# JacekNaruniec/LiveScan3D

Hardware: AMD Instinct MI355X
Metric: fused frames/s (N x 512x424 depth -> merged cloud) (higher is better)
Workload: dtype f32

## Files before the change

### livescan3d_amd/csrc/fusion.hip

```cpp


#include "fusion_shared.hpp"

namespace {

struct Iv { float lo, hi; };
__device__ __forceinline__ Iv iv_scale(Iv a, float c) { const float x = a.lo * c, y = a.hi * c; return c >= 0.0f ? Iv{x, y} : Iv{y, x}; }
__device__ __forceinline__ Iv iv_shift(Iv a, float c) { return Iv{a.lo + c, a.hi + c}; }
__device__ __forceinline__ Iv iv_sum(Iv a, Iv b) { return Iv{a.lo + b.lo, a.hi + b.hi}; }
__device__ __forceinline__ bool iv_finite(Iv a) { return isfinite(a.lo) && isfinite(a.hi); }

__device__ __forceinline__ float depth_to_metres1(float d)
{
    const f2 z = depth_to_metres2(f2{d, d});
    return z.x;
}

__device__ __forceinline__ int classify_range(int a, int b, float xfac, float yfac, const SensorParams &P, const float (&bx)[6])
{
    if (a == b) {
        f2 ox, oy, oz;
        unproject2(f2{(float)a, (float)a}, f2{xfac, xfac}, f2{yfac, yfac}, P, ox, oy, oz);
        const bool rejected = (ox.x < bx[0]) | (ox.x > bx[3]) | (oy.x < bx[1]) | (oy.x > bx[4]) | (oz.x < bx[2]) | (oz.x > bx[5]);
        return rejected ? 0 : 1;
// ... 51 lines not shown
    }
}

template <bool VEC>
__device__ __forceinline__ void load_thresholds(const FuseArgs &a, const Tile &t, unsigned int (&lo)[kPxPerLane], unsigned int (&cnt)[kPxPerLane],
                                                bool &any_flagged)
{
    const int p0 = t.px0 + threadIdx.x * kPxPerLane;
    unsigned int c[kPxPerLane];
#pragma unroll
    for (int k = 0; k < kPxPerLane; k++) c[k] = 1u;
    const unsigned int *tp = a.thr + t.pix_base + p0;
    if (VEC) {
        if (p0 < t.npix) {
            const uint4 u = reinterpret_cast<const uint4 *>(tp)[0], v = reinterpret_cast<const uint4 *>(tp)[1];
            c[0] = u.x; c[1] = u.y; c[2] = u.z; c[3] = u.w; c[4] = v.x; c[5] = v.y; c[6] = v.z; c[7] = v.w;
        }
    } else {
#pragma unroll
        for (int k = 0; k < kPxPerLane; k++)
            if (p0 + k < t.npix) c[k] = tp[k];
    }
    bool fl = false;
#pragma unroll
    for (int k = 0; k < kPxPerLane; k++) {
        lo[k] = c[k] & 0xFFFFu;
        cnt[k] = c[k] >> 16;
        fl |= lo[k] == 0;
    }
    any_flagged = __any(fl);
}

__device__ __forceinline__ int wave_count_thr(const Inputs &in, const unsigned int (&lo)[kPxPerLane], const unsigned int (&cnt)[kPxPerLane])
{
    int wt = 0;
#pragma unroll
    for (int k = 0; k < kPxPerLane; k++) {
        const unsigned int d = (k & 1) ? in.dw[k >> 1] >> 16 : in.dw[k >> 1] & 0xFFFFu;
        wt += __popcll(__ballot(d - lo[k] < cnt[k]));
    }
    return wt;
}

template <bool VEC, int kTickGroup>
__global__ __launch_bounds__(kThreads) void count_thr_kernel(const FuseArgs a)
{
    __shared__ int s_cnt[4][kTickGroup];
    const int lane = threadIdx.x & 63;
    const int wave = threadIdx.x >> 6;
    const int tg = blockIdx.x / a.tiles_per_tick;
    const int tile = blockIdx.x - tg * a.tiles_per_tick;
    const int tick0 = tg * kTickGroup;
    const int nt = min(kTickGroup, a.n_ticks - tick0);
    const Tile t = locate(a, tick0, tile);
    unsigned int lo[kPxPerLane], cnt[kPxPerLane];
    bool any_flagged;
    load_thresholds<VEC>(a, t, lo, cnt, any_flagged);
    Inputs in[kTickGroup];
#pragma unroll
    for (int i = 0; i < kTickGroup; i++) {
        Tile ti = t;
        ti.dptr = t.dptr + (long long)(i < nt ? i : 0) * a.tick_depth_stride;
        load_inputs<VEC, false>(ti, in[i]);
    }
    if (!any_flagged) {
#pragma unroll
        for (int i = 0; i < kTickGroup; i++) {
            const int wt = wave_count_thr(in[i], lo, cnt);
            if (lane == 0) s_cnt[wave][i] = wt;
        }
    } else {
        const SensorParams P = a.params[t.f];
        float xf[kPxPerLane], yf[kPxPerLane];
        tile_factors<VEC>(t, xf, yf);
#pragma unroll 1
        for (int i = 0; i < nt; i++) {
            Tile ti = t;
            ti.dptr = t.dptr + (long long)i * a.tick_depth_stride;
            Inputs ix;
            load_inputs<VEC, false>(ti, ix);
            bool keep[kPxPerLane];
            uint4 unused[kPxPerLane];
            compute_pixels<false>(a, P, ix, xf, yf, keep, unused);
            int wt = 0;
#pragma unroll
            for (int k = 0; k < kPxPerLane; k++) wt += __popcll(__ballot(keep[k]));
            if (lane == 0) s_cnt[wave][i] = wt;
        }
    }
    __syncthreads();
    if ((int)threadIdx.x < nt)
        a.tile_counts[(long long)(tick0 + threadIdx.x) * a.tiles_per_tick + tile] =
            s_cnt[0][threadIdx.x] + s_cnt[1][threadIdx.x] + s_cnt[2][threadIdx.x] + s_cnt[3][threadIdx.x];
}

constexpr unsigned long long kFlagAggregate = 1ull << 62;
constexpr unsigned long long kFlagPrefix = 2ull << 62;
constexpr int kSpinLimit = 1 << 20;

constexpr int kEpochShift = 34;
constexpr unsigned long long kTileAggregate = 1ull << 32, kTilePrefix = 2ull << 32;

__device__ __forceinline__ int tile_lookback(const FuseArgs &a, int tick, int tile, int tile_tot, int lane)
{
    unsigned long long *st = a.run_state + (long long)tick * a.tiles_per_tick;
    const unsigned long long tag = (unsigned long long)a.epoch << kEpochShift;
    if (lane == 0)
        __hip_atomic_store(&st[tile], tag | (tile == 0 ? kTilePrefix : kTileAggregate) | (unsigned int)tile_tot, __ATOMIC_RELAXED,
                           __HIP_MEMORY_SCOPE_AGENT);
    int acc = 0;
    int pos = tile - 1 - lane;
    bool done = tile == 0;
    int spins = 0;
    const bool near_polls = a.n_ticks > 1;
    while (!done) {
        unsigned long long w = tag | kTilePrefix;
        if (pos >= 0) {
            if (near_polls && (spins & 3) != 3) w = __hip_atomic_load(&st[pos], __ATOMIC_RELAXED, __HIP_MEMORY_SCOPE_WORKGROUP);
            else w = __hip_atomic_load(&st[pos], __ATOMIC_RELAXED, __HIP_MEMORY_SCOPE_AGENT);
        }
        bool again = false;
        const unsigned int flag = (w >> kEpochShift) == a.epoch ? (unsigned int)(w >> 32) & 3u : 0u;
        const unsigned long long pref = __ballot(flag == 2);
        const int first = pref ? __ffsll((long long)pref) - 1 : 63;
        const unsigned long long relevant = first >= 63 ? ~0ull : ((2ull << first) - 1ull);
        const bool poisoned = (__ballot(flag == 3) & relevant) != 0;
        if (poisoned || (__ballot(flag == 0) & relevant) != 0) {
            if (poisoned || ++spins > kSpinLimit) {
                if (lane == 0) {
                    atomicExch(a.error_flag, 1);
                    if (a.offsets_mirror) a.offsets_mirror[a.n_frames + 1] = 1;
                    __hip_atomic_store(&st[tile], tag | (3ull << 32), __ATOMIC_RELAXED, __HIP_MEMORY_SCOPE_AGENT);
                }
                return -1;
            }
            __builtin_amdgcn_s_sleep(1);
            again = true;
        } else {
            acc += wave_sum(lane <= first ? (int)(unsigned int)w : 0);
            if (pref) done = true;
        }
        if (!done && !again) pos -= 64;
    }
    if (lane == 0 && tile != 0)
        __hip_atomic_store(&st[tile], tag | kTilePrefix | (unsigned int)(acc + tile_tot), __ATOMIC_RELAXED, __HIP_MEMORY_SCOPE_AGENT);
    return acc;
}


template <int MODE, bool VEC, bool LAZY = false, bool HOST = false>
__global__ __launch_bounds__(kThreads) void fuse_kernel(const FuseArgs a)
{
    constexpr bool kWrite = MODE != 0;
    __shared__ uint4 stage[kWrite ? kStageSlots : 1];
    __shared__ int s_wave_tot[4];
    __shared__ int s_wave_next[4];
    __shared__ int s_base;
    const int lane = threadIdx.x & 63;
    const int wave = threadIdx.x >> 6;
    int tick = blockIdx.x / a.tiles_per_tick;
    int tile = blockIdx.x - tick * a.tiles_per_tick;
    if (kWrite && a.chunk > 0) {
        const int per_chunk = a.chunk * a.n_ticks;
        const int chunk = blockIdx.x / per_chunk;
        const int r = blockIdx.x - chunk * per_chunk;
        const int width = min(a.chunk, a.tiles_per_tick - chunk * a.chunk);
        tick = r / width;
        tile = chunk * a.chunk + (r - tick * width);
    }
    tile += a.tile0;
    if (MODE == 1 && a.reverse_ticks) tick = a.n_ticks - 1 - tick;
    const int lin = tick * a.tiles_per_tick + tile;

    const Tile t = locate(a, tick, tile);
    Inputs in;
    load_inputs<VEC, kWrite && !LAZY>(t, in);
    Inputs nx;
    if (MODE == 3) {
        Tile tn = t;
        tn.dptr = a.depth_next + tick * a.tick_depth_stride + t.pix_base;
        load_inputs<VEC, false>(tn, nx);
    }
    const SensorParams P = a.params[t.f];
    float xf[kPxPerLane], yf[kPxPerLane];
    tile_factors<VEC>(t, xf, yf);
    bool keep[kPxPerLane];
    uint4 vert[kPxPerLane];
    compute_pixels<kWrite>(a, P, in, xf, yf, keep, vert);
    if (kWrite && LAZY) {
        bool any = false;
#pragma unroll
        for (int k = 0; k < kPxPerLane; k++) any |= keep[k];
        if (any) {
            load_rgb<VEC>(t, in);
#pragma unroll
            for (int k = 0; k < kPxPerLane; k++) vert[k].x = rgba_of(in, k);
        }
    }
    if (MODE == 3) {
        int wt = 0;
        bool arithmetic = true;
        if (a.thr) {
            unsigned int lo[kPxPerLane], cnt[kPxPerLane];
            bool any_flagged;
            load_thresholds<VEC>(a, t, lo, cnt, any_flagged);
            arithmetic = any_flagged;
            if (!any_flagged) wt = wave_count_thr(nx, lo, cnt);
        }
        if (arithmetic) {
            bool keep_n[kPxPerLane];
            uint4 unused[kPxPerLane];
            compute_pixels<false>(a, P, nx, xf, yf, keep_n, unused);
#pragma unroll
            for (int k = 0; k < kPxPerLane; k++) wt += __popcll(__ballot(keep_n[k]));
        }
        if (lane == 0) s_wave_next[wave] = wt;
    }

    int below, wave_total;
    rank_from_masks(keep, below, wave_total);
    if (lane == 0) s_wave_tot[wave] = wave_total;
    int base = 0, counted = 0;
    if (MODE == 1 || MODE == 3) {
        base = a.tile_counts[lin];
        counted = (tile + 1 < a.tiles_per_tick ? a.tile_counts[lin + 1] : a.offsets[tick * (a.n_frames + 1) + a.n_frames]) - base;
    }
    __syncthreads();
    int wave_off = 0, tile_tot = 0;
#pragma unroll
    for (int i = 0; i < 4; i++) {
        const int v = s_wave_tot[i];
        if (i < wave) wave_off += v;
        tile_tot += v;
    }
    if (MODE == 0) {
        if (threadIdx.x == 0) a.tile_counts[lin] = tile_tot;
        return;
    }
    if (MODE == 3 && threadIdx.x == 0) a.tile_counts_next[lin] = s_wave_next[0] + s_wave_next[1] + s_wave_next[2] + s_wave_next[3];
    if (MODE == 4) {
        if (wave == 0) {
            const int b = tile_lookback(a, tick, tile, tile_tot, lane);
            if (lane == 0) s_base = b;
        }
        __syncthreads();
        base = s_base;
        if (base < 0) {
            if (threadIdx.x == 0 && tile == a.tiles_per_tick - 1) {
                a.offsets[tick * (a.n_frames + 1) + a.n_frames] = -1;
                if (a.offsets_mirror) a.offsets_mirror[a.n_frames] = -1;
            }
            return;
        }
        if (threadIdx.x == 0) {
            int *off = a.offsets + tick * (a.n_frames + 1);
            if (t.frame_start) off[t.f] = base;
            if (tile == a.tiles_per_tick - 1) off[a.n_frames] = base + tile_tot;
            if (a.offsets_mirror) {
                if (t.frame_start) a.offsets_mirror[t.f] = base;
                if (tile == a.tiles_per_tick - 1) a.offsets_mirror[a.n_frames] = base + tile_tot;
            }
            if (a.group_end_mirror && blockIdx.x == gridDim.x - 1) *a.group_end_mirror = base + tile_tot;
        }
    }
    if (MODE != 4 && tile_tot != counted) {
        if (threadIdx.x == 0) atomicExch(a.error_flag, 2);
        return;
    }
    if (VEC ? a.pm_first != nullptr : a.pixmap != nullptr) {
        const int p0 = t.px0 + threadIdx.x * kPxPerLane;
        if (p0 < t.npix) {
            int r = base + wave_off + below;
            if (VEC) {
                unsigned int m = 0;
#pragma unroll
                for (int k = 0; k < kPxPerLane; k++) m |= keep[k] ? (1u << k) : 0u;
                const long long g = (tick * a.tick_depth_stride + t.pix_base + p0) >> 3;
                a.pm_first[g] = r;
                a.pm_mask[g] = (unsigned char)m;
            } else {
                int *pm = a.pixmap + tick * a.tick_depth_stride + t.pix_base + p0;
#pragma unroll
                for (int k = 0; k < kPxPerLane; k++) {
                    if (p0 + k < t.npix) pm[k] = keep[k] ? r : -1;
                    r += keep[k] ? 1 : 0;
                }
            }
        }
    }
    stage_and_store(stage, keep, vert, wave_off + below, tile_tot, a.out + tick * a.tick_vert_stride + base, HOST || (MODE == 4 && a.host_out != 0));
}



template <bool VEC>
__global__ __launch_bounds__(kThreads) void run_kernel(const FuseArgs a)
{
    __shared__ uint4 stage[kStageSlots];
    __shared__ int s_wave_tot[4];
    __shared__ int s_run;
    __shared__ int s_base;
    const int lane = threadIdx.x & 63;
    const int wave = threadIdx.x >> 6;

    const int tick = blockIdx.x % a.n_ticks;
    if (threadIdx.x == 0) s_run = (int)atomicAdd(a.ticket + 32 * tick, 1u);
    __syncthreads();
    const int run = s_run;
    if (run >= a.runs_per_tick) return;
    const int t0 = run * a.tiles_per_run;
    const int t1 = min(t0 + a.tiles_per_run, a.tiles_per_tick);

    int wave_total = 0;
    {
        Tile t = locate(a, tick, t0);
        Inputs in;
        load_inputs<VEC, false>(t, in);
        for (int tile = t0; tile < t1; tile++) {
            Tile tn = t;
            Inputs nx = in;
            if (tile + 1 < t1) {
                tn = locate(a, tick, tile + 1);
                load_inputs<VEC, false>(tn, nx);
            }
            bool counted = false;
            if (a.thr) {
                unsigned int lo[kPxPerLane], cnt[kPxPerLane];
                bool any_flagged;
                load_thresholds<VEC>(a, t, lo, cnt, any_flagged);
                if (!any_flagged) {
                    wave_total += wave_count_thr(in, lo, cnt);
                    counted = true;
                }
            }
            if (!counted) {
                bool keep[kPxPerLane];
                uint4 unused[kPxPerLane];
                compute_tile<VEC, false>(a, t, in, keep, unused);
#pragma unroll
                for (int k = 0; k < kPxPerLane; k++) wave_total += __popcll(__ballot(keep[k]));
            }
            t = tn;
            in = nx;
        }
    }
    if (lane == 0) s_wave_tot[wave] = wave_total;
    __syncthreads();
    const int run_tot = s_wave_tot[0] + s_wave_tot[1] + s_wave_tot[2] + s_wave_tot[3];

    Tile t = locate(a, tick, t0);
    Inputs in;
    load_inputs<VEC, true>(t, in);

    if (wave == 0) {
        unsigned long long *st = a.run_state + (long long)tick * a.tiles_per_tick;
        if (lane == 0) {
            const unsigned long long w = (run == 0 ? kFlagPrefix : kFlagAggregate) | (unsigned int)run_tot;
            __hip_atomic_store(&st[run], w, __ATOMIC_RELAXED, __HIP_MEMORY_SCOPE_AGENT);
        }
        int acc = 0;
        int pos = run - 1 - lane;
        bool done = run == 0;
        int spins = 0;
        while (!done) {
            unsigned long long w = kFlagPrefix;
            if (pos >= 0) w = __hip_atomic_load(&st[pos], __ATOMIC_RELAXED, __HIP_MEMORY_SCOPE_AGENT);
            const unsigned int flag = (unsigned int)(w >> 62);
            const unsigned long long pref = __ballot(flag == 2);
            const int first = pref ? __ffsll((long long)pref) - 1 : 63;
            const unsigned long long relevant = first >= 63 ? ~0ull : ((2ull << first) - 1ull);
            const unsigned long long empty = __ballot(flag == 0) & relevant;
            if (empty != 0) {
                if (++spins > kSpinLimit) {
                    if (lane == 0) atomicExch(a.error_flag, 1);
                    break;
                }
                __builtin_amdgcn_s_sleep(2);
                continue;
            }
            const int v = (lane <= first) ? (int)(unsigned int)w : 0;
            acc += wave_sum(v);
            if (pref) done = true;
            else pos -= 64;
        }
        if (lane == 0) {
            if (run != 0) {
                const unsigned long long w = kFlagPrefix | (unsigned int)(acc + run_tot);
                __hip_atomic_store(&st[run], w, __ATOMIC_RELAXED, __HIP_MEMORY_SCOPE_AGENT);
            }
            s_base = acc;
        }
    }
    __syncthreads();
    int running = s_base;

    int *off = a.offsets + (long long)tick * (a.n_frames + 1);
    for (int tile = t0; tile < t1; tile++) {
        Tile tn = t;
        Inputs nx = in;
        if (tile + 1 < t1) {
            tn = locate(a, tick, tile + 1);
            load_inputs<VEC, true>(tn, nx);
        }
        bool keep[kPxPerLane];
        uint4 vert[kPxPerLane];
        compute_tile<VEC, true>(a, t, in, keep, vert);
        int below, wave_tot2;
        rank_from_masks(keep, below, wave_tot2);
        if (lane == 0) s_wave_tot[wave] = wave_tot2;
        __syncthreads();
        int wave_off = 0, tile_tot = 0;
#pragma unroll
        for (int i = 0; i < 4; i++) {
            const int v = s_wave_tot[i];
            if (i < wave) wave_off += v;
            tile_tot += v;
        }
        if (threadIdx.x == 0 && t.frame_start) off[t.f] = running;
        if (tile_tot > 0) {
            stage_and_store(stage, keep, vert, wave_off + below, tile_tot, a.out + tick * a.tick_vert_stride + running);
        } else {
            __syncthreads();
        }
        running += tile_tot;
        t = tn;
        in = nx;
    }
    if (threadIdx.x == 0 && t1 == a.tiles_per_tick) off[a.n_frames] = running;
}


__global__ __launch_bounds__(kThreads) void table_kernel(const FrameDesc *frames, const SensorParams *params, int n_frames, float *xtab,
                                                         float *ytab)
{
    const int f = blockIdx.y;
    if (f >= n_frames) return;
    const FrameDesc fd = frames[f];
    const SensorParams P = params[f];
    for (int i = blockIdx.x * kThreads + threadIdx.x; i < fd.w + fd.h; i += gridDim.x * kThreads) {
        if (i < fd.w) xtab[fd.xtab_off + i] = ((float)i - P.cx) / P.fx;
        else ytab[fd.ytab_off + (i - fd.w)] = (P.cy - (float)(i - fd.w)) / P.fy;
    }
}
// ... 109 lines not shown
        for (auto &e : p->events) {
            (void)hipEventDestroy(e.first);
            (void)hipEventDestroy(e.second);
        }
        p->rd.destroy_event();
        if (p->side) {
            (void)hipStreamSynchronize(p->side);
            (void)hipStreamDestroy(p->side);
            (void)hipEventDestroy(p->ev_counted);
            (void)hipEventDestroy(p->ev_written[0]);
            (void)hipEventDestroy(p->ev_written[1]);
        }
        delete p;
    });
}

extern "C" long long lsnFusionTickCapacity(const LsnFusion *p) { return p ? p->cap : 0; }

extern "C" int lsnPackSensorParams(const float *intr7, const float *wt12, float *out16)
{
    return lsn::guarded("lsnPackSensorParams", -1, [&]() {
        lsn::clear_error();
        if (!intr7 || !wt12 || !out16) {
            lsn::set_error("lsnPackSensorParams: null argument");
            return -1;
        }
        SensorParams s;
        pack_sensor_params(intr7, wt12, s);
        static_assert(sizeof(SensorParams) == 16 * sizeof(float), "SensorParams is 16 floats");
        memcpy(out16, &s, sizeof(s));
        return 0;
    });
}

extern "C" int lsnFusionSetParams(LsnFusion *p, const float *intr, const float *wt, const float *bounds6, void *stream)
{
    return lsn::guarded("lsnFusionSetParams", -1, [&]() {
        lsn::clear_error();
        if (!p || !intr || !wt || !bounds6) {
            lsn::set_error("lsnFusionSetParams: null argument");
            return -1;
        }
        LSN_HIP(hipSetDevice(p->device));
        {
            std::lock_guard<std::mutex> g(p->mu);
            if (p->params_set && p->last_intr.size() == 7 * (size_t)p->n_maps &&
                memcmp(p->last_intr.data(), intr, sizeof(float) * 7 * p->n_maps) == 0 &&
                memcmp(p->last_wt.data(), wt, sizeof(float) * 12 * p->n_maps) == 0 && memcmp(p->bounds, bounds6, sizeof(p->bounds)) == 0)
                return 0;
        }
        std::vector<SensorParams> sp(p->n_maps);
        for (int i = 0; i < p->n_maps; i++) pack_sensor_params(intr + 7 * i, wt + 12 * i, sp[i]);
        LSN_HIP(hipMemcpyAsync(p->params.p, sp.data(), sizeof(SensorParams) * p->n_maps, hipMemcpyHostToDevice,
                               lsn::as_stream(stream)));
        hipLaunchKernelGGL(table_kernel, dim3(8, (unsigned)p->n_maps), dim3(kThreads), 0, lsn::as_stream(stream), p->frames.as<FrameDesc>(),
                           p->params.as<SensorParams>(), p->n_maps, p->xtab.as<float>(), p->ytab.as<float>());
        LSN_HIP(hipGetLastError());
        LSN_HIP(hipStreamSynchronize(lsn::as_stream(stream)));
        std::lock_guard<std::mutex> g(p->mu);
        memcpy(p->bounds, bounds6, sizeof(p->bounds));
        p->last_intr.assign(intr, intr + 7 * (size_t)p->n_maps);
        p->last_wt.assign(wt, wt + 12 * (size_t)p->n_maps);
        p->params_set = true;
        p->params_gen++;
        p->thr_valid = false;
        p->runs_with_params = 0;
        return 0;
    });
}

extern "C" int lsnFusionSetMode(LsnFusion *p, int mode)
{
    return lsn::guarded("lsnFusionSetMode", -1, [&]() {
        if (!p || mode < lsn::kPlanThreeLaunches || mode > lsn::kPlanSinglePass) {
            lsn::set_error("lsnFusionSetMode: mode must be 0 (count/scan/write launches), 1 (single launch, runs + look-back) or 2 (single pass, look-back per tile)");
            return -1;
        }
        p->mode = mode;
        return 0;
    });
}

extern "C" int lsnFusionSetPipelined(LsnFusion *p, int enable)
{
    return lsn::guarded("lsnFusionSetPipelined", -1, [&]() {
        lsn::clear_error();
        if (!p) return -1;
        std::lock_guard<std::mutex> g(p->mu);
        LSN_HIP(hipSetDevice(p->device));
        if (enable && !p->side) {
            if (p->tile_counts_b.reserve(sizeof(int) * (size_t)p->tiles_per_tick * p->n_ticks) ||
                p->offs_int.reserve(sizeof(int) * 2 * (size_t)p->n_ticks * (p->n_maps + 1)))
                return -1;
            LSN_HIP(hipStreamCreateWithFlags(&p->side, hipStreamNonBlocking));
            LSN_HIP(hipEventCreateWithFlags(&p->ev_counted, hipEventDisableTiming));
            LSN_HIP(hipEventCreateWithFlags(&p->ev_written[0], hipEventDisableTiming));
            LSN_HIP(hipEventCreateWithFlags(&p->ev_written[1], hipEventDisableTiming));
        }
        if (!enable && p->side) LSN_HIP(hipStreamSynchronize(p->side));
        p->pipelined = enable != 0;
        p->calls = 0;
        return 0;
    });
}

extern "C" int lsnFusionProfile(LsnFusion *p, int enable)
{
    return lsn::guarded("lsnFusionProfile", -1, [&]() {
        if (!p) return -1;
        p->profile = enable != 0;
        p->profile_every = enable > 1 ? enable : 1;
        p->profile_seq = 0;
        return 0;
    });
}

static int drain_events(LsnFusion *p)
{
    for (size_t i = 0; i < p->ev_used; i++) {
        float ms = 0;
        LSN_HIP(hipEventSynchronize(p->events[i].second));
        LSN_HIP(hipEventElapsedTime(&ms, p->events[i].first, p->events[i].second));
        p->acc_ms += ms;
        p->launches++;
    }
    p->ev_used = 0;
    return 0;
}

extern "C" int lsnFusionKernelStats(LsnFusion *p, double *avg_ms, long long *launches, char *name, int name_len, int reset)
{
    return lsn::guarded("lsnFusionKernelStats", -1, [&]() {
        lsn::clear_error();
        if (!p) return -1;
        std::lock_guard<std::mutex> g(p->mu);
        LSN_HIP(hipSetDevice(p->device));
        if (drain_events(p)) return -1;
        if (avg_ms) *avg_ms = p->launches ? p->acc_ms / (double)p->launches : 0.0;
        if (launches) *launches = p->launches;
        if (name && name_len > 0)
            snprintf(name, (size_t)name_len, "%s", p->timed_kernel ? p->timed_kernel : (p->mode == lsn::kPlanThreeLaunches ? "fuse_kernel<1>" : p->mode == lsn::kPlanSinglePass ? "fuse_kernel<4>" : "run_kernel"));
        if (reset) {
            p->acc_ms = 0;
            p->launches = 0;
        }
        return 0;
    });
}

void lsn::fill_args(LsnFusion *p, FuseArgs &a, const void *d_depth, const void *d_colors, void *d_vertices, int *d_offsets, bool with_pixmap)
{
    a.epoch = 0;
    a.chunk = 0;
    a.frames = p->frames.as<FrameDesc>();
    a.tiles = p->tile_frame.as<TileDesc>();
    a.params = p->params.as<SensorParams>();
    a.xtab = p->xtab.as<float>();
    a.ytab = p->ytab.as<float>();
    a.depth = static_cast<const unsigned short *>(d_depth);
    a.rgb = static_cast<const unsigned char *>(d_colors);
    a.out = static_cast<uint4 *>(d_vertices);
    a.tile_counts = p->tile_counts.as<int>();
    a.run_state = p->tile_state.as<unsigned long long>();
    a.error_flag = p->misc.as<int>();
    a.ticket = p->misc.as<unsigned int>() + 32;
    a.offsets = d_offsets;
    a.pixmap = with_pixmap ? p->pixmap.as<int>() : nullptr;
    a.pm_first = with_pixmap ? p->pm_first.as<int>() : nullptr;
    a.pm_mask = with_pixmap ? p->pm_mask.as<unsigned char>() : nullptr;
    a.n_frames = p->n_maps;
    a.tiles_per_tick = p->tiles_per_tick;
    a.n_ticks = p->n_ticks;
    {
        const long long total = (long long)p->tiles_per_tick * p->n_ticks;
        long long tpr = total / (6ll * 7 * 256);
        if (tpr < 1) tpr = 1;
        if (tpr > 8) tpr = 8;
        if (tpr > p->tiles_per_tick) tpr = p->tiles_per_tick;
        a.tiles_per_run = (int)tpr;
        a.runs_per_tick = (p->tiles_per_tick + a.tiles_per_run - 1) / a.tiles_per_run;
    }
    a.tick_depth_stride = p->tick_depth_elems;
    a.tick_rgb_stride = p->tick_rgb_bytes;
    a.tick_vert_stride = p->cap;
    a.minX = p->bounds[0]; a.minY = p->bounds[1]; a.minZ = p->bounds[2];
    a.maxX = p->bounds[3]; a.maxY = p->bounds[4]; a.maxZ = p->bounds[5];

    a.depth_next = nullptr;
    a.tile_counts_next = nullptr;
    a.thr = p->thr_valid ? p->thr.as<unsigned int>() : nullptr;
    a.tile0 = 0;
    a.reverse_ticks = 1;
    a.host_out = 0;
    a.offsets_mirror = nullptr;
    a.group_end_mirror = nullptr;
}

int lsn::ensure_thresholds(LsnFusion *p, hipStream_t s)
{
    if (!p->thr_enabled || p->thr_valid) return 0;
    if (++p->runs_with_params < 2) return 0;
    if (p->thr.reserve(sizeof(unsigned int) * (size_t)p->cap)) return -1;
    hipEvent_t e0, e1;
    LSN_HIP(hipEventCreate(&e0));
    LSN_HIP(hipEventCreate(&e1));
    LSN_HIP(hipEventRecord(e0, s));
    hipLaunchKernelGGL(thresh_kernel, dim3(256, (unsigned)p->n_maps), dim3(kThreads), 0, s, p->frames.as<FrameDesc>(), p->params.as<SensorParams>(),
                       p->n_maps, p->xtab.as<float>(), p->ytab.as<float>(), p->thr.as<unsigned int>(), p->bounds[0], p->bounds[1], p->bounds[2],
                       p->bounds[3], p->bounds[4], p->bounds[5]);
    LSN_HIP(hipGetLastError());
    LSN_HIP(hipEventRecord(e1, s));
    LSN_HIP(hipEventSynchronize(e1));
    (void)hipEventElapsedTime(&p->thr_build_ms, e0, e1);
    (void)hipEventDestroy(e0);
    (void)hipEventDestroy(e1);
    p->thr_valid = true;
    return 0;
}

template <int MODE, bool LAZY, bool HOST>
static void launch_fuse_as(bool vec, int grid, hipStream_t s, const FuseArgs &a)
{
    if (vec) hipLaunchKernelGGL((fuse_kernel<MODE, true, LAZY, HOST>), dim3(grid), dim3(kThreads), 0, s, a);
    else     hipLaunchKernelGGL((fuse_kernel<MODE, false, LAZY, HOST>), dim3(grid), dim3(kThreads), 0, s, a);
}

template <int MODE>
static void launch_fuse(bool vec, int grid, hipStream_t s, const FuseArgs &a, bool lazy_rgb = false, bool host_out = false)
{
    if constexpr (MODE == lsn::kPassWrite) {
        if (host_out) return launch_fuse_as<MODE, true, true>(vec, grid, s, a);
    }
    if constexpr (MODE == lsn::kPassWrite || MODE == lsn::kPassSingle) {
        if (lazy_rgb) return launch_fuse_as<MODE, true, false>(vec, grid, s, a);
    }
    launch_fuse_as<MODE, false, false>(vec, grid, s, a);
}

template <int kTickGroup>
static void launch_count_thr(bool vec, int grid, hipStream_t s, const FuseArgs &a)
{
    if (vec) hipLaunchKernelGGL((count_thr_kernel<true, kTickGroup>), dim3(grid), dim3(kThreads), 0, s, a);
    else     hipLaunchKernelGGL((count_thr_kernel<false, kTickGroup>), dim3(grid), dim3(kThreads), 0, s, a);
}

void lsn::count_and_scan(LsnFusion *p, bool vec, hipStream_t s, const FuseArgs &a, int *mirror)
{
    if (a.thr) {
        const int G = a.n_ticks >= 8 ? 8 : (a.n_ticks >= 4 ? 4 : 1);
        const int grid = p->tiles_per_tick * ((a.n_ticks + G - 1) / G);
        if (G == 8) launch_count_thr<8>(vec, grid, s, a);
        else if (G == 4) launch_count_thr<4>(vec, grid, s, a);
        else launch_count_thr<1>(vec, grid, s, a);
    } else {
        launch_fuse<lsn::kPassCount>(vec, p->tiles_per_tick * a.n_ticks, s, a);
    }
    hipLaunchKernelGGL(scan_kernel, dim3((unsigned)a.n_ticks), dim3(kScanThreads), 0, s, a.tile_counts, a.tiles_per_tick, a.frames, a.n_frames, a.offsets, mirror);
}

int lsn::next_event_pair(LsnFusion *p, hipEvent_t &e0, hipEvent_t &e1)
{
    if (p->ev_used == p->events.size()) {
        if (p->events.size() >= 4096) {
            if (drain_events(p)) return -1;
        } else {
            hipEvent_t x, y;
            LSN_HIP(hipEventCreate(&x));
            LSN_HIP(hipEventCreate(&y));
            p->events.emplace_back(x, y);
        }
    }
    e0 = p->events[p->ev_used].first;
    e1 = p->events[p->ev_used].second;
    p->ev_used++;
    return 0;
}

extern "C" int lsnFusionRun(LsnFusion *p, const void *d_depth, const void *d_colors, void *d_vertices, int *d_offsets,
                            void *stream)
{
    return lsn::guarded("lsnFusionRun", -1, [&]() {
        lsn::clear_error();
        return lsn::run_vertices(p, d_depth, d_colors, d_vertices, d_offsets, lsn::as_stream(stream));
    });
}

int lsn::run_vertices(LsnFusion *p, const void *d_depth, const void *d_colors, void *d_vertices, int *d_offsets, hipStream_t s)
{
    if (!p || !d_depth || !d_colors || !d_vertices || !d_offsets) {
        lsn::set_error("lsnFusionRun: null argument");
        return -1;
    }
    std::lock_guard<std::mutex> g(p->mu);
    return lsn::run_locked(p, d_depth, d_colors, d_vertices, d_offsets, s, false);
}

static int next_epoch(LsnFusion *p, hipStream_t s)
{
    if (p->epoch == 0 || p->epoch >= (1u << 30) - 1) {
        LSN_HIP(hipMemsetAsync(p->tile_state.p, 0, sizeof(unsigned long long) * (size_t)p->tiles_per_tick * p->n_ticks, s));
        p->epoch = 0;
    }
    ++p->epoch;
    return 0;
}


static int run_three_launches(LsnFusion *p, FuseArgs &a, bool vec, hipStream_t s, hipEvent_t e0, hipEvent_t e1)
{
    count_and_scan(p, vec, s, a);
    if (e0) LSN_HIP(hipEventRecord(e0, s));
    a.chunk = 0;
    launch_fuse<lsn::kPassWrite>(vec, p->tiles_per_tick * p->n_ticks, s, a, p->lazy_rgb);
    if (e1) LSN_HIP(hipEventRecord(e1, s));
    return 0;
}

static int run_pipelined(LsnFusion *p, FuseArgs &a, bool vec, hipStream_t s, hipEvent_t e0, hipEvent_t e1)
{
    const int b = (int)(p->calls & 1);
    const size_t off_elems = (size_t)p->n_ticks * (p->n_maps + 1);
    int *d_offsets = a.offsets, *off_int = p->offs_int.as<int>() + b * off_elems;
    a.tile_counts = b ? p->tile_counts_b.as<int>() : p->tile_counts.as<int>();
    if (p->calls >= 2) LSN_HIP(hipStreamWaitEvent(p->side, p->ev_written[b], 0));
    a.offsets = off_int;
    count_and_scan(p, vec, p->side, a);
    a.offsets = d_offsets;
    LSN_HIP(hipEventRecord(p->ev_counted, p->side));
    LSN_HIP(hipStreamWaitEvent(s, p->ev_counted, 0));
    LSN_HIP(hipMemcpyAsync(d_offsets, off_int, sizeof(int) * off_elems, hipMemcpyDeviceToDevice, s));
    if (e0) LSN_HIP(hipEventRecord(e0, s));
    launch_fuse<lsn::kPassWrite>(vec, p->tiles_per_tick * p->n_ticks, s, a);
    if (e1) LSN_HIP(hipEventRecord(e1, s));
    LSN_HIP(hipEventRecord(p->ev_written[b], s));
    p->calls++;
    return 0;
}

static int run_single_pass(LsnFusion *p, FuseArgs &a, bool vec, hipStream_t s, hipEvent_t e0, hipEvent_t e1)
{
    if (next_epoch(p, s)) return -1;
    a.epoch = p->epoch;
    constexpr int kFuseChunk = 16;
    a.chunk = kFuseChunk;
    if (e0) LSN_HIP(hipEventRecord(e0, s));
    launch_fuse<lsn::kPassSingle>(vec, p->tiles_per_tick * p->n_ticks, s, a, p->lazy_rgb);
    if (e1) LSN_HIP(hipEventRecord(e1, s));
    return 0;
}

static int run_lookback_runs(LsnFusion *p, FuseArgs &a, bool vec, hipStream_t s, hipEvent_t e0, hipEvent_t e1)
{
    LSN_HIP(hipMemsetAsync(p->tile_state.p, 0, sizeof(unsigned long long) * (size_t)p->tiles_per_tick * p->n_ticks, s));
    LSN_HIP(hipMemsetAsync(p->misc.as<char>() + 128, 0, 128 * (size_t)p->n_ticks, s));
    if (e0) LSN_HIP(hipEventRecord(e0, s));
    const int rgrid = a.runs_per_tick * p->n_ticks;
    if (vec) hipLaunchKernelGGL((run_kernel<true>), dim3(rgrid), dim3(kThreads), 0, s, a);
    else     hipLaunchKernelGGL((run_kernel<false>), dim3(rgrid), dim3(kThreads), 0, s, a);
    if (e1) LSN_HIP(hipEventRecord(e1, s));
    return 0;
}

enum class RunForm { ThreeLaunches, Pipelined, SinglePass, LookbackRuns };
static RunForm run_form(const LsnFusion *p, bool with_pixmap)
{
    switch (p->mode) {
    case lsn::kPlanThreeLaunches:
        if (p->pipelined) return with_pixmap ? RunForm::ThreeLaunches : RunForm::Pipelined;
        return p->n_ticks == 1 && p->one_tick_single_pass ? RunForm::SinglePass : RunForm::ThreeLaunches;
    case lsn::kPlanLookbackRuns:
        return with_pixmap ? RunForm::ThreeLaunches : RunForm::LookbackRuns;
    default:
        return with_pixmap ? RunForm::ThreeLaunches : RunForm::SinglePass;
    }
}

int lsn::run_locked(LsnFusion *p, const void *d_depth, const void *d_colors, void *d_vertices, int *d_offsets, hipStream_t s, bool with_pixmap)
{
    if (!p->params_set) {
        lsn::set_error("lsnFusionRun: lsnFusionSetParams has not been called");
        return -1;
    }
    if (((uintptr_t)d_vertices & 15) != 0) {
        lsn::set_error("lsnFusionRun: d_vertices must be 16-byte aligned");
        return -1;
    }
    LSN_HIP(hipSetDevice(p->device));
    if (ensure_thresholds(p, s)) return -1;
    FuseArgs a;
    fill_args(p, a, d_depth, d_colors, d_vertices, d_offsets, with_pixmap);
    const bool vec = wide_loads(p, d_depth, d_colors);

    hipEvent_t e0 = nullptr, e1 = nullptr;
    if (timed_launch(p) && next_event_pair(p, e0, e1)) return -1;

    const RunForm form = run_form(p, with_pixmap);
    if (p->mode == lsn::kPlanThreeLaunches) p->timed_kernel = form == RunForm::SinglePass ? "fuse_kernel<4>" : nullptr;
    int rc = -1;
    switch (form) {
    case RunForm::ThreeLaunches: rc = run_three_launches(p, a, vec, s, e0, e1); break;
    case RunForm::Pipelined:     rc = run_pipelined(p, a, vec, s, e0, e1); break;
    case RunForm::SinglePass:    rc = run_single_pass(p, a, vec, s, e0, e1); break;
    case RunForm::LookbackRuns:  rc = run_lookback_runs(p, a, vec, s, e0, e1); break;
    }
    if (rc) return -1;
    LSN_HIP(hipGetLastError());
    return 0;
}

int lsn::run_frames(LsnFusion *p, const void *d_depth, const void *d_colors, void *d_vertices, int *d_offsets, int f0, int f1, bool first_of_tick,
                    bool with_pixmap, int *offsets_mirror, int *group_end_mirror, bool host_out, hipStream_t s)
{
    if (!p || !d_depth || !d_colors || !d_vertices || !d_offsets || f0 < 0 || f1 > p->n_maps || f0 >= f1 || p->n_ticks != 1) {
        lsn::set_error("run_frames: bad arguments");
        return -1;
    }
    if (!p->params_set) {
        lsn::set_error("run_frames: lsnFusionSetParams has not been called");
        return -1;
    }
    std::lock_guard<std::mutex> g(p->mu);
    LSN_HIP(hipSetDevice(p->device));
    const bool vec = wide_loads(p, d_depth, d_colors);
    if (with_pixmap && reserve_pixmap(p, vec)) return -1;
    FuseArgs a;
    fill_args(p, a, d_depth, d_colors, d_vertices, d_offsets, with_pixmap);
    if (first_of_tick && next_epoch(p, s)) return -1;
    a.epoch = p->epoch;
    a.chunk = 0;
    a.tile0 = p->tile_start[f0];
    a.offsets_mirror = offsets_mirror;
    a.group_end_mirror = group_end_mirror;
    a.host_out = host_out ? 1 : 0;
    launch_fuse<lsn::kPassSingle>(vec, p->tile_start[f1] - p->tile_start[f0], s, a, p->lazy_rgb);
    LSN_HIP(hipGetLastError());
    return 0;
}

int lsn::run_count(LsnFusion *p, const void *d_depth, const void *d_colors, int *d_offsets, int *offsets_mirror, hipEvent_t counted, hipStream_t s)
{
    if (!p || !d_depth || !d_colors || !d_offsets || p->n_ticks != 1) {
        lsn::set_error("run_count: bad arguments");
        return -1;
    }
    if (!p->params_set) {
        lsn::set_error("run_count: lsnFusionSetParams has not been called");
        return -1;
    }
    std::lock_guard<std::mutex> g(p->mu);
    LSN_HIP(hipSetDevice(p->device));
    if (ensure_thresholds(p, s)) return -1;
    FuseArgs a;
    fill_args(p, a, d_depth, d_colors, nullptr, d_offsets, false);
    count_and_scan(p, wide_loads(p, d_depth, d_colors), s, a, offsets_mirror);
    LSN_HIP(hipGetLastError());
    if (counted) LSN_HIP(hipEventRecord(counted, s));
    return 0;
}

int lsn::run_write(LsnFusion *p, const void *d_depth, const void *d_colors, void *vertices, int *d_offsets, bool with_pixmap, bool host_out, hipStream_t s)
{
    if (!p || !d_depth || !d_colors || !vertices || !d_offsets || p->n_ticks != 1 || ((uintptr_t)vertices & 15) != 0) {
        lsn::set_error("run_write: bad arguments");
        return -1;
    }
    std::lock_guard<std::mutex> g(p->mu);
    LSN_HIP(hipSetDevice(p->device));
    const bool vec = wide_loads(p, d_depth, d_colors);
    if (with_pixmap && reserve_pixmap(p, vec)) return -1;
    FuseArgs a;
    fill_args(p, a, d_depth, d_colors, vertices, d_offsets, with_pixmap);
    launch_fuse<lsn::kPassWrite>(vec, p->tiles_per_tick, s, a, p->lazy_rgb, host_out);
    LSN_HIP(hipGetLastError());
    return 0;
}

extern "C" int lsnFusionRunStreamed(LsnFusion *p, const void *d_depth, const void *d_colors, void *d_vertices, int *d_offsets,
                                    const void *d_next_depth, void *stream)
{
    return lsn::guarded("lsnFusionRunStreamed", -1, [&]() {
        lsn::clear_error();
        if (!p || !d_depth || !d_colors || !d_vertices || !d_offsets) {
            lsn::set_error("lsnFusionRunStreamed: null argument");
            return -1;
        }
        if (!p->params_set) {
            lsn::set_error("lsnFusionRunStreamed: lsnFusionSetParams has not been called");
            return -1;
        }
        std::lock_guard<std::mutex> g(p->mu);
        LSN_HIP(hipSetDevice(p->device));
        hipStream_t s = lsn::as_stream(stream);
        const size_t n_tiles = (size_t)p->tiles_per_tick * p->n_ticks;
        const size_t off_elems = (size_t)p->n_ticks * (p->n_maps + 1);
        if (p->tile_counts_b.reserve(sizeof(int) * n_tiles) || p->offs_int.reserve(sizeof(int) * 2 * off_elems)) return -1;

        if (ensure_thresholds(p, s)) return -1;
// ... 80 lines not shown
```

### livescan3d_amd/csrc/fusion_shared.hpp

```cpp
#pragma once

#include "lsn_common.hpp"
#include "wave_ops.hpp"

#include <cstdint>
#include <mutex>
#include <vector>

namespace lsn {

constexpr int kPlanThreeLaunches = 0;
constexpr int kPlanLookbackRuns = 1;
constexpr int kPlanSinglePass = 2;
constexpr int kPassCount = 0;
constexpr int kPassWrite = 1;
constexpr int kPassWriteCountNext = 3;
constexpr int kPassSingle = 4;

struct FrameDesc {
    int w, h, npix, tile_start;
    long long depth_off;
    long long rgb_off;
    int xtab_off, ytab_off;
    float inv_w;
    int pad1;
};

struct TileDesc {
    int frame;
    int x0, y0;
    int pad;
};

struct SensorParams {
    float cx, cy, fx, fy;
    float t0, t1, t2;
    float r00, r01, r02, r10, r11, r12, r20, r21, r22;
};

inline void pack_sensor_params(const float *ip, const float *tp, SensorParams &s)
{
    s.cx = ip[0]; s.cy = ip[1]; s.fx = ip[2]; s.fy = ip[3];
    s.t0 = tp[0]; s.t1 = tp[1]; s.t2 = tp[2];
    s.r00 = tp[3]; s.r01 = tp[4]; s.r02 = tp[5];
    s.r10 = tp[6]; s.r11 = tp[7]; s.r12 = tp[8];
    s.r20 = tp[9]; s.r21 = tp[10]; s.r22 = tp[11];
}

struct FuseArgs {
    const FrameDesc *frames;
    const TileDesc *tiles;
    const SensorParams *params;
    const float *xtab;
    const float *ytab;
    const unsigned short *depth;
    const unsigned char *rgb;
    uint4 *out;
    int *tile_counts;
    unsigned long long *run_state;
    unsigned int *ticket;
    int *offsets;
    int *pixmap;
    int *pm_first;
    unsigned char *pm_mask;
    const unsigned short *depth_next;
    int *tile_counts_next;
    int *error_flag;
    const unsigned int *thr;
    int n_frames;
    int tiles_per_tick;
    int n_ticks;
    int tiles_per_run;
    unsigned int epoch;
    int chunk;
    int reverse_ticks;
    int tile0;
    int host_out;
    int *group_end_mirror;
    int *offsets_mirror;
    int runs_per_tick;
    long long tick_depth_stride;
    long long tick_rgb_stride;
    long long tick_vert_stride;
    float minX, minY, minZ, maxX, maxY, maxZ;
};

struct TriArgs {
    const FrameDesc *frames;
    const TileDesc *tiles;
    const unsigned short *depth;
    const int *pixmap;
    const int *pm_first;
    const unsigned char *pm_mask;
    int *tri;
    int *tile_counts;
    unsigned int *codes;
    int tiles_per_tick;
    int win;
    int host_out;
    int index_base;
    long long tick_pix_stride;
    long long tick_tri_stride;
};

}
using lsn::FrameDesc;
using lsn::FuseArgs;
using lsn::TriArgs;
using lsn::SensorParams;
using lsn::pack_sensor_params;
using lsn::TileDesc;

namespace {

constexpr int kThreads = 256;
constexpr int kPxPerLane = 8;
constexpr int kTile = kThreads * kPxPerLane;
constexpr int kWin = 1152;
constexpr bool kNontemporalStores = true;



typedef float f2 __attribute__((ext_vector_type(2)));

__device__ __forceinline__ f2 depth_to_metres2(f2 d)
{
    const f2 r = {0x1.0624dep-10f, 0x1.0624dep-10f};
    const f2 k = {1000.0f, 1000.0f};
    const f2 q0 = d * r;
    const f2 e = __builtin_elementwise_fma(-q0, k, d);
    return __builtin_elementwise_fma(e, r, q0);
}

__device__ __forceinline__ void unproject2(f2 d, f2 xfac, f2 yfac, const SensorParams &P, f2 &ox, f2 &oy, f2 &oz)
{
    f2 Z = depth_to_metres2(d);
    f2 X = xfac * Z;
    f2 Y = yfac * Z;
    X = X + P.t0;
    Y = Y + P.t1;
    Z = Z + P.t2;
    ox = X * P.r00 + Y * P.r01 + Z * P.r02;
    oy = X * P.r10 + Y * P.r11 + Z * P.r12;
    oz = X * P.r20 + Y * P.r21 + Z * P.r22;
}

__device__ __forceinline__ bool inside_box(float ox, float oy, float oz, const FuseArgs &a)
{
    const bool rejected = (ox < a.minX) | (ox > a.maxX) | (oy < a.minY) | (oy > a.maxY) | (oz < a.minZ) | (oz > a.maxZ);
    return !rejected;
}

__device__ __forceinline__ void rank_from_masks(const bool (&keep)[kPxPerLane], int &below, int &wave_total)
{
    below = 0;
    wave_total = 0;
#pragma unroll
    for (int k = 0; k < kPxPerLane; k++) {
        const unsigned long long m = __ballot(keep[k]);
        below = __builtin_amdgcn_mbcnt_hi((unsigned int)(m >> 32), __builtin_amdgcn_mbcnt_lo((unsigned int)m, below));
        wave_total += __popcll(m);
    }
}


struct Tile {
    long long pix_base;
    int f, w, h, npix, px0;
    int x0, y0;
    float inv_w;
    bool frame_start;
    const unsigned short *dptr;
    const unsigned char *cptr;
    const float *xt, *yt;
};

__device__ __forceinline__ Tile locate(const FuseArgs &a, int tick, int tile)
{
    Tile t;
    const TileDesc td = a.tiles[tile];
    t.f = td.frame;
    t.x0 = td.x0;
    t.y0 = td.y0;
    const FrameDesc fd = a.frames[t.f];
    t.inv_w = fd.inv_w;
    t.pix_base = fd.depth_off;
    t.w = fd.w;
    t.h = fd.h;
    t.npix = fd.npix;
    t.px0 = (tile - fd.tile_start) * kTile;
    t.frame_start = tile == fd.tile_start;
    t.dptr = a.depth + tick * a.tick_depth_stride + fd.depth_off;
    t.cptr = a.rgb + tick * a.tick_rgb_stride + fd.rgb_off;
    t.xt = a.xtab + fd.xtab_off;
    t.yt = a.ytab + fd.ytab_off;
    return t;
}

struct Inputs {
    unsigned int dw[4];
    unsigned int cw[6];
};

template <bool VEC, bool RGB>
__device__ __forceinline__ void load_inputs(const Tile &t, Inputs &in)
{
    const int p0 = t.px0 + threadIdx.x * kPxPerLane;
#pragma unroll
    for (int i = 0; i < 4; i++) in.dw[i] = 0;
#pragma unroll
    for (int i = 0; i < 6; i++) in.cw[i] = 0;
    if (VEC) {
        if (p0 < t.npix) {
            const uint4 dv = *reinterpret_cast<const uint4 *>(t.dptr + p0);
            in.dw[0] = dv.x; in.dw[1] = dv.y; in.dw[2] = dv.z; in.dw[3] = dv.w;
            if (RGB) {
                const uint2 *cp = reinterpret_cast<const uint2 *>(t.cptr + 3ll * p0);
                const uint2 c0 = cp[0], c1 = cp[1], c2 = cp[2];
                in.cw[0] = c0.x; in.cw[1] = c0.y; in.cw[2] = c1.x; in.cw[3] = c1.y; in.cw[4] = c2.x; in.cw[5] = c2.y;
            }
        }
    } else {
#pragma unroll
        for (int k = 0; k < kPxPerLane; k++) {
            if (p0 + k < t.npix) {
                const unsigned int d = t.dptr[p0 + k];
                in.dw[k >> 1] |= d << ((k & 1) * 16);
                if (RGB) {
                    const unsigned char *c = t.cptr + 3ll * (p0 + k);
                    const unsigned int rgb = c[0] | (c[1] << 8) | (c[2] << 16);
                    const int b = 3 * k;
                    in.cw[b >> 2] |= rgb << ((b & 3) * 8);
                    if ((b & 3) > 1) in.cw[(b >> 2) + 1] |= rgb >> ((4 - (b & 3)) * 8);
                }
            }
        }
    }
}

template <bool VEC>
__device__ __forceinline__ void load_rgb(const Tile &t, Inputs &in)
{
    const int p0 = t.px0 + threadIdx.x * kPxPerLane;
    if (VEC) {
        if (p0 < t.npix) {
            const uint2 *cp = reinterpret_cast<const uint2 *>(t.cptr + 3ll * p0);
            const uint2 c0 = cp[0], c1 = cp[1], c2 = cp[2];
            in.cw[0] = c0.x; in.cw[1] = c0.y; in.cw[2] = c1.x; in.cw[3] = c1.y; in.cw[4] = c2.x; in.cw[5] = c2.y;
        }
    } else {
#pragma unroll
        for (int k = 0; k < kPxPerLane; k++) {
            if (p0 + k < t.npix) {
                const unsigned char *c = t.cptr + 3ll * (p0 + k);
                const unsigned int rgb = c[0] | (c[1] << 8) | (c[2] << 16);
                const int b = 3 * k;
                in.cw[b >> 2] |= rgb << ((b & 3) * 8);
                if ((b & 3) > 1) in.cw[(b >> 2) + 1] |= rgb >> ((4 - (b & 3)) * 8);
            }
        }
    }
}

__device__ __forceinline__ unsigned int rgba_of(const Inputs &in, int k)
{
    const int b = 3 * k;
    const unsigned int lo = in.cw[b >> 2];
    const unsigned int hi = in.cw[(b >> 2) + 1 < 6 ? (b >> 2) + 1 : 5];
    return (__funnelshift_r(lo, hi, (b & 3) * 8) & 0x00FFFFFFu) | 0xFF000000u;
}

__device__ __forceinline__ void lane_origin(const Tile &t, int &x, int &y)
{
    const int p0 = t.px0 + threadIdx.x * kPxPerLane;
    const int v = t.x0 + (int)threadIdx.x * kPxPerLane;
    int q = (int)((float)v * t.inv_w);
    x = v - q * t.w;
    if (x < 0) { q--; x += t.w; }
    if (x >= t.w) { q++; x -= t.w; }
    y = t.y0 + q;
    if (p0 >= t.npix) { x = 0; y = 0; }
}

__device__ __forceinline__ void store_vertex(uint4 *dst, const uint4 v)
{
    if (kNontemporalStores) {
        __builtin_nontemporal_store(v.x, &dst->x);
        __builtin_nontemporal_store(v.y, &dst->y);
        __builtin_nontemporal_store(v.z, &dst->z);
        __builtin_nontemporal_store(v.w, &dst->w);
    } else {
        *dst = v;
    }
}

template <bool VEC>
__device__ __forceinline__ void tile_factors(const Tile &t, float (&xf)[kPxPerLane], float (&yf)[kPxPerLane])
{
    int x, y;
    lane_origin(t, x, y);
    float yfac = t.yt[y];
    if (VEC) {
        const float4 x0 = *reinterpret_cast<const float4 *>(t.xt + x);
        const float4 x1 = *reinterpret_cast<const float4 *>(t.xt + x + 4);
        xf[0] = x0.x; xf[1] = x0.y; xf[2] = x0.z; xf[3] = x0.w;
        xf[4] = x1.x; xf[5] = x1.y; xf[6] = x1.z; xf[7] = x1.w;
#pragma unroll
        for (int k = 0; k < kPxPerLane; k++) yf[k] = yfac;
    } else {
#pragma unroll
        for (int k = 0; k < kPxPerLane; k++) {
            xf[k] = t.xt[x];
            yf[k] = yfac;
            x++;
            if (x == t.w) {
                x = 0;
                y = y + 1 < t.h ? y + 1 : y;
                yfac = t.yt[y];
            }
        }
    }
}

template <bool WRITE>
__device__ __forceinline__ void compute_pixels(const FuseArgs &a, const SensorParams &P, const Inputs &in, const float (&xf)[kPxPerLane],
                                               const float (&yf)[kPxPerLane], bool (&keep)[kPxPerLane], uint4 (&vert)[kPxPerLane])
{
#pragma unroll
    for (int k = 0; k < kPxPerLane; k += 2) {
        const unsigned int d0 = in.dw[k >> 1] & 0xFFFFu, d1 = in.dw[k >> 1] >> 16;
        f2 ox, oy, oz;
        unproject2(f2{(float)d0, (float)d1}, f2{xf[k], xf[k + 1]}, f2{yf[k], yf[k + 1]}, P, ox, oy, oz);
        keep[k] = inside_box(ox.x, oy.x, oz.x, a) && d0 != 0;
        keep[k + 1] = inside_box(ox.y, oy.y, oz.y, a) && d1 != 0;
        if (WRITE) {
#pragma unroll
            for (int j = 0; j < 2; j++) {
                vert[k + j].x = rgba_of(in, k + j);
                vert[k + j].y = __float_as_uint(j ? ox.y : ox.x);
                vert[k + j].z = __float_as_uint(j ? oy.y : oy.x);
                vert[k + j].w = __float_as_uint(j ? oz.y : oz.x);
            }
        }
    }
}

template <bool VEC, bool WRITE>
__device__ __forceinline__ void compute_tile(const FuseArgs &a, const Tile &t, const Inputs &in, bool (&keep)[kPxPerLane],
                                             uint4 (&vert)[kPxPerLane])
{
    const SensorParams P = a.params[t.f];
    float xf[kPxPerLane], yf[kPxPerLane];
    tile_factors<VEC>(t, xf, yf);
    compute_pixels<WRITE>(a, P, in, xf, yf, keep, vert);
}

constexpr int kStagePadShift = 3;
__device__ __forceinline__ int stage_slot16(int q) { return q + (q >> kStagePadShift); }
constexpr int kStageSlots = kWin + (kWin >> kStagePadShift) + 1;

__device__ __forceinline__ void stage_and_store(uint4 *stage, const bool (&keep)[kPxPerLane], const uint4 (&vert)[kPxPerLane], int rank0,
                                                int tile_tot, uint4 *dst, bool host_dst = false)
{
    for (int w0 = 0; w0 < tile_tot; w0 += kWin) {
        int r = rank0 - w0;
#pragma unroll
        for (int k = 0; k < kPxPerLane; k++) {
            if (keep[k]) {
                if ((unsigned int)r < (unsigned int)kWin) stage[stage_slot16(r)] = vert[k];
                r++;
            }
        }
        __syncthreads();
        const int n = min(kWin, tile_tot - w0);
        if (host_dst) {
            const int mis = (int)((reinterpret_cast<uintptr_t>(dst + w0) >> 4) & 63);
            for (int i = (int)threadIdx.x - mis; i < n; i += kThreads)
                if (i >= 0) dst[w0 + i] = stage[stage_slot16(i)];
        } else
        for (int i = threadIdx.x; i < n; i += kThreads) {
            const uint4 v = stage[stage_slot16(i)];
            if (kNontemporalStores) {
                __builtin_nontemporal_store(v.x, &dst[w0 + i].x);
                __builtin_nontemporal_store(v.y, &dst[w0 + i].y);
                __builtin_nontemporal_store(v.z, &dst[w0 + i].z);
                __builtin_nontemporal_store(v.w, &dst[w0 + i].w);
            } else {
                dst[w0 + i] = v;
            }
        }
        __syncthreads();
    }
}

template <int ELEM, typename T>
__device__ __forceinline__ void store_run(T *dst, const T *lds, int lead, int n)
{
    static_assert(sizeof(T) == ELEM, "element size");
    const int end = lead + n;
    const int c0 = lead ? 1 : 0, c1 = end >> 4;
    uint4 *g16 = reinterpret_cast<uint4 *>(reinterpret_cast<unsigned char *>(dst) - lead);
    const uint4 *l16 = reinterpret_cast<const uint4 *>(lds);
    for (int j = c0 + (int)threadIdx.x; j < c1; j += kThreads) g16[j] = l16[j];
    const int head = lead ? min(n, 16 - lead) : 0;
    const int tail0 = max(head, 16 * c1 - lead);
    const int t = (int)threadIdx.x * ELEM;
    if (t < head) dst[threadIdx.x] = lds[lead / ELEM + threadIdx.x];
    if (tail0 + t < n) dst[tail0 / ELEM + threadIdx.x] = lds[(lead + tail0) / ELEM + threadIdx.x];
}

constexpr int kScanThreads = 1024;
constexpr int kScanItems = 8;
constexpr int kScanWaves = kScanThreads / 64;

__device__ __forceinline__ void scan_tick(int *tc, int tiles_per_tick, const FrameDesc *frames, int n_frames, int *off, int *mirror_row,
                                          int (&s_wave)[kScanWaves])
{
    const int lane = threadIdx.x & 63, wave = threadIdx.x >> 6;
    int carry = 0;
    for (int c0 = 0; c0 < tiles_per_tick; c0 += kScanThreads * kScanItems) {
        const int i0 = c0 + (int)threadIdx.x * kScanItems;
        int v[kScanItems];
        const bool whole = i0 + kScanItems <= tiles_per_tick && (reinterpret_cast<uintptr_t>(tc + i0) & 15) == 0;
        if (whole) {
            const int4 a = reinterpret_cast<const int4 *>(tc + i0)[0], b = reinterpret_cast<const int4 *>(tc + i0)[1];
            v[0] = a.x; v[1] = a.y; v[2] = a.z; v[3] = a.w; v[4] = b.x; v[5] = b.y; v[6] = b.z; v[7] = b.w;
        } else {
#pragma unroll
            for (int k = 0; k < kScanItems; k++) v[k] = i0 + k < tiles_per_tick ? tc[i0 + k] : 0;
        }
        int t = 0;
#pragma unroll
        for (int k = 0; k < kScanItems; k++) {
            const int x = v[k];
            v[k] = t;
            t += x;
        }
        const int incl = wave_scan_incl(t, lane);
        if (lane == 63) s_wave[wave] = incl;
        __syncthreads();
        int pre = carry, round_tot = 0;
#pragma unroll
        for (int w = 0; w < kScanWaves; w++) {
            const int x = s_wave[w];
            if (w < wave) pre += x;
            round_tot += x;
        }
        pre += incl - t;
        if (whole) {
            reinterpret_cast<int4 *>(tc + i0)[0] = make_int4(pre + v[0], pre + v[1], pre + v[2], pre + v[3]);
            reinterpret_cast<int4 *>(tc + i0)[1] = make_int4(pre + v[4], pre + v[5], pre + v[6], pre + v[7]);
        } else {
#pragma unroll
            for (int k = 0; k < kScanItems; k++)
                if (i0 + k < tiles_per_tick) tc[i0 + k] = pre + v[k];
        }
        carry += round_tot;
        __syncthreads();
    }
    for (int f = threadIdx.x; f <= n_frames; f += kScanThreads) {
        const int v = f < n_frames ? tc[frames[f].tile_start] : carry;
        off[f] = v;
        if (mirror_row) mirror_row[f] = v;
    }
}

__attribute__((unused)) __global__ __launch_bounds__(kScanThreads) void scan_kernel(int *tile_counts, int tiles_per_tick, const FrameDesc *frames, int n_frames,
                                                        int *offsets, int *mirror)
{
    __shared__ int s_wave[kScanWaves];
    const int tick = blockIdx.x;
    scan_tick(tile_counts + (long long)tick * tiles_per_tick, tiles_per_tick, frames, n_frames, offsets + (long long)tick * (n_frames + 1),
                     mirror ? mirror + (long long)tick * (n_frames + 1) : nullptr, s_wave);
}


}


struct LsnFusion {
    int device = 0;
    int n_ticks = 0, n_maps = 0;
    std::vector<int> w, h;
    std::vector<int> tile_start;
    long long cap = 0;
    long long tick_depth_elems = 0, tick_rgb_bytes = 0;
    int tiles_per_tick = 0;
    bool vec_ok = false;
    bool params_set = false;
    int mode = lsn::kPlanThreeLaunches;
    unsigned int epoch = 0;
    float bounds[6] = {0, 0, 0, 0, 0, 0};
    lsn::DevBuf frames, tile_frame, params, tile_counts, tile_state, misc;
    lsn::DevBuf xtab, ytab;
    lsn::DevBuf pixmap, pm_first, pm_mask, tri_counts, tri_codes;
    bool pixmap_compact = false;
    lsn::RadialScratch rd;
    bool pipelined = false;
    hipStream_t side = nullptr;
    hipEvent_t ev_counted = nullptr, ev_written[2] = {nullptr, nullptr};
    lsn::DevBuf tile_counts_b, offs_int;
    unsigned long long calls = 0;
    const void *counted_for = nullptr;
    unsigned long long counted_gen = 0, params_gen = 1;
    int stream_half = 0;
    lsn::DevBuf thr;
    lsn::DevBuf ix_counts, ix_off, ix_pix2v, ix_v2pix, ix_conf, ix_ctile;
    bool ix_conf_ready = false;
    lsn::DevBuf ct_cov, ct_pairs, ct_blk, ct_stats, ct_samples, ct_xform;
    bool ct_ready = false;
    int ct_nblk = 0;
    lsn::DevBuf mg_toff, mg_depth0, mg_depth, mg_d2v, mg_assigned, mg_vconf, mg_proj, mg_zmax, mg_key, mg_mdepth, mg_mtag, mg_ero;
    bool mg_ready = false;
    lsn::DevBuf ol_key, ol_bucket, ol_chunk, ol_pts, ol_removed, ol_stats, ol_offs, ol_tab, ol_box, ol_frame;
    bool ol_ready = false;
    int ol_nb = 0, ol_nchunk = 0;
    lsn::DevBuf fl_tiles, fl_counts;
    std::vector<int> fl_tile_frame;
    bool fl_ready = false;
    int fl_tiles_per_tick = 0;
    int fl_last = 0;
    hipStream_t fl_stream = nullptr;
    int ds_radius = 0, ds_n_range = 0;
    std::vector<unsigned short> ds_table_host;
    lsn::DevBuf ds_table, ds_counts;
    int ds_last = 0;
    hipStream_t ds_stream = nullptr;
// ... 53 lines not shown
```

Baseline: 221,500.

## Overlap lazy RGB loads with lookback and regroup single-pass block order

In the single-pass fuse kernel, the RGB fetch and RGBA packing now run after the tile count is known, issued alongside the decoupled lookback wait, so the load latency can hide behind the inter-block prefix chain. Block scheduling now groups ticks, up to 64 at a time, with a smaller tile chunk of 8, which changes the order in which tiles across frames are dispatched. The staging window for single-pass shrinks to 1024 slots to reduce shared memory per block and may raise occupancy. The trade-off is extra index arithmetic, and tiles with more than 1024 kept points may need additional store windows.

```diff
diff --git a/livescan3d_amd/csrc/fusion.hip b/livescan3d_amd/csrc/fusion.hip
--- a/livescan3d_amd/csrc/fusion.hip
+++ b/livescan3d_amd/csrc/fusion.hip
@@ -227,7 +227,9 @@
 __global__ __launch_bounds__(kThreads) void fuse_kernel(const FuseArgs a)
 {
     constexpr bool kWrite = MODE != 0;
-    __shared__ uint4 stage[kWrite ? kStageSlots : 1];
+    constexpr bool kSingle = MODE == 4;
+    constexpr int kWindow = kSingle ? kWinSingle : kWin;
+    __shared__ uint4 stage[kWrite ? stage_slots(kWindow) : 1];
     __shared__ int s_wave_tot[4];
     __shared__ int s_wave_next[4];
     __shared__ int s_base;
@@ -236,12 +238,18 @@
     int tick = blockIdx.x / a.tiles_per_tick;
     int tile = blockIdx.x - tick * a.tiles_per_tick;
     if (kWrite && a.chunk > 0) {
-        const int per_chunk = a.chunk * a.n_ticks;
-        const int chunk = blockIdx.x / per_chunk;
-        const int r = blockIdx.x - chunk * per_chunk;
+        const int per_group = a.tick_group * a.tiles_per_tick;
+        const int group = blockIdx.x / per_group;
+        const int rg = blockIdx.x - group * per_group;
+        const int tick0 = group * a.tick_group;
+        const int gticks = min(a.tick_group, a.n_ticks - tick0);
+        const int per_chunk = a.chunk * gticks;
+        const int chunk = rg / per_chunk;
+        const int r = rg - chunk * per_chunk;
         const int width = min(a.chunk, a.tiles_per_tick - chunk * a.chunk);
-        tick = r / width;
-        tile = chunk * a.chunk + (r - tick * width);
+        const int gt = r / width;
+        tick = tick0 + gt;
+        tile = chunk * a.chunk + (r - gt * width);
     }
     tile += a.tile0;
     if (MODE == 1 && a.reverse_ticks) tick = a.n_ticks - 1 - tick;
@@ -261,8 +269,8 @@
     tile_factors<VEC>(t, xf, yf);
     bool keep[kPxPerLane];
     uint4 vert[kPxPerLane];
-    compute_pixels<kWrite>(a, P, in, xf, yf, keep, vert);
-    if (kWrite && LAZY) {
+    compute_pixels<kWrite, kWrite && !kSingle>(a, P, in, xf, yf, keep, vert);
+    if (kWrite && LAZY && !kSingle) {
         bool any = false;
 #pragma unroll
         for (int k = 0; k < kPxPerLane; k++) any |= keep[k];
@@ -314,9 +322,20 @@
     }
     if (MODE == 3 && threadIdx.x == 0) a.tile_counts_next[lin] = s_wave_next[0] + s_wave_next[1] + s_wave_next[2] + s_wave_next[3];
     if (MODE == 4) {
+        bool any = true;
+        if (LAZY) {
+            any = false;
+#pragma unroll
+            for (int k = 0; k < kPxPerLane; k++) any |= keep[k];
+            if (any) load_rgb<VEC>(t, in);
+        }
         if (wave == 0) {
             const int b = tile_lookback(a, tick, tile, tile_tot, lane);
             if (lane == 0) s_base = b;
+        }
+        if (any) {
+#pragma unroll
+            for (int k = 0; k < kPxPerLane; k++) vert[k].x = rgba_of(in, k);
         }
         __syncthreads();
         base = s_base;
@@ -363,7 +382,7 @@
             }
         }
     }
-    stage_and_store(stage, keep, vert, wave_off + below, tile_tot, a.out + tick * a.tick_vert_stride + base, HOST || (MODE == 4 && a.host_out != 0));
+    stage_and_store<kWindow>(stage, keep, vert, wave_off + below, tile_tot, a.out + tick * a.tick_vert_stride + base, HOST || (MODE == 4 && a.host_out != 0));
 }
 
 
@@ -779,6 +798,7 @@
 {
     a.epoch = 0;
     a.chunk = 0;
+    a.tick_group = p->n_ticks;
     a.frames = p->frames.as<FrameDesc>();
     a.tiles = p->tile_frame.as<TileDesc>();
     a.params = p->params.as<SensorParams>();
@@ -968,8 +988,10 @@
 {
     if (next_epoch(p, s)) return -1;
     a.epoch = p->epoch;
-    constexpr int kFuseChunk = 16;
+    constexpr int kFuseChunk = 8;
+    constexpr int kFuseTickGroup = 64;
     a.chunk = kFuseChunk;
+    a.tick_group = std::min(p->n_ticks, kFuseTickGroup);
     if (e0) LSN_HIP(hipEventRecord(e0, s));
     launch_fuse<lsn::kPassSingle>(vec, p->tiles_per_tick * p->n_ticks, s, a, p->lazy_rgb);
     if (e1) LSN_HIP(hipEventRecord(e1, s));
diff --git a/livescan3d_amd/csrc/fusion_shared.hpp b/livescan3d_amd/csrc/fusion_shared.hpp
--- a/livescan3d_amd/csrc/fusion_shared.hpp
+++ b/livescan3d_amd/csrc/fusion_shared.hpp
@@ -73,6 +73,7 @@
     int tiles_per_run;
     unsigned int epoch;
     int chunk;
+    int tick_group;
     int reverse_ticks;
     int tile0;
     int host_out;
@@ -117,6 +118,7 @@
 constexpr int kPxPerLane = 8;
 constexpr int kTile = kThreads * kPxPerLane;
 constexpr int kWin = 1152;
+constexpr int kWinSingle = 1024;
 constexpr bool kNontemporalStores = true;
 
 
@@ -322,7 +324,7 @@
     }
 }
 
-template <bool WRITE>
+template <bool WRITE, bool RGBA = WRITE>
 __device__ __forceinline__ void compute_pixels(const FuseArgs &a, const SensorParams &P, const Inputs &in, const float (&xf)[kPxPerLane],
                                                const float (&yf)[kPxPerLane], bool (&keep)[kPxPerLane], uint4 (&vert)[kPxPerLane])
 {
@@ -336,7 +338,7 @@
         if (WRITE) {
 #pragma unroll
             for (int j = 0; j < 2; j++) {
-                vert[k + j].x = rgba_of(in, k + j);
+                if (RGBA) vert[k + j].x = rgba_of(in, k + j);
                 vert[k + j].y = __float_as_uint(j ? ox.y : ox.x);
                 vert[k + j].z = __float_as_uint(j ? oy.y : oy.x);
                 vert[k + j].w = __float_as_uint(j ? oz.y : oz.x);
@@ -357,22 +359,24 @@
 
 constexpr int kStagePadShift = 3;
 __device__ __forceinline__ int stage_slot16(int q) { return q + (q >> kStagePadShift); }
-constexpr int kStageSlots = kWin + (kWin >> kStagePadShift) + 1;
-
+constexpr int stage_slots(int win) { return win + (win >> kStagePadShift) + 1; }
+constexpr int kStageSlots = stage_slots(kWin);
+
+template <int WIN = kWin>
 __device__ __forceinline__ void stage_and_store(uint4 *stage, const bool (&keep)[kPxPerLane], const uint4 (&vert)[kPxPerLane], int rank0,
                                                 int tile_tot, uint4 *dst, bool host_dst = false)
 {
-    for (int w0 = 0; w0 < tile_tot; w0 += kWin) {
+    for (int w0 = 0; w0 < tile_tot; w0 += WIN) {
         int r = rank0 - w0;
 #pragma unroll
         for (int k = 0; k < kPxPerLane; k++) {
             if (keep[k]) {
-                if ((unsigned int)r < (unsigned int)kWin) stage[stage_slot16(r)] = vert[k];
+                if ((unsigned int)r < (unsigned int)WIN) stage[stage_slot16(r)] = vert[k];
                 r++;
             }
         }
         __syncthreads();
-        const int n = min(kWin, tile_tot - w0);
+        const int n = min(WIN, tile_tot - w0);
         if (host_dst) {
             const int mis = (int)((reinterpret_cast<uintptr_t>(dst + w0) >> 4) & 63);
             for (int i = (int)threadIdx.x - mis; i < n; i += kThreads)
```

Result: no change. 222,100 (median of 4 runs) (+0.3%).
